# aligirayhanozbay/poisson_CNN

Measured on AMD Instinct MI355X. Metric: grids/sec (fwd+bwd) at 1024^2, higher is better.
Workload: dtype f32; 1 GPU; c4: Homogeneous_Poisson_NN_Legacy(hpnn.json) full train step (fwd+bwd+loss+Adam), 8 x 1024x1024 Dirichlet grids per GPU; global_batch=8, parallelism=dp1, math=fp32, ranks_seen=1

## Files before the change

### poisson_cnn_amd/csrc/conv_small.hip

```cpp
#include "pcnn_internal.h"
#include "conv_epilogue.h"

int pcnn_conv_small_fwd(pcnn_handle h, const pcnn_conv_desc* d, const float* x, const float* w, const float* bias, const float* bn_scale,
                        const float* bn_shift, const float* residual, float* y, float* act_out);
int pcnn_conv_small_wgrad(pcnn_handle h, const pcnn_conv_desc* d, const float* x, const float* dz, float* dw, void* workspace, size_t workspace_bytes);
bool pcnn_conv_fwd_takes_narrow_route(pcnn_handle h, const pcnn_conv_desc* d);
bool pcnn_conv_small_fwd_eligible(const pcnn_conv_desc* d);
bool pcnn_conv_small_wgrad_eligible(const pcnn_conv_desc* d);
size_t pcnn_conv_small_wgrad_workspace(const pcnn_conv_desc* d);

namespace {

constexpr int STH = 8, STW = 32;
__host__ __device__ constexpr int lds_stride(int CI) { return CI == 16 ? 20 : CI; }

struct SmallParams {
  const float* x; const float* wp; const float* bias; const float* bn_scale; const float* bn_shift; const float* res; float* y; float* act_out;
  unsigned* absmax;
  int N, H, W, Cin, ldx, Ho, Wo, Cout, ldy, pt, pl, pad_mode; float pad_value; int act; float alpha;
  int ld_res, ld_act, tiles_x, tiles_y, vec_in, vec_out;
  const float* gact = nullptr; float* y2 = nullptr; float* bpart = nullptr;
  int ld_gact = 0, ld_y2 = 0, gmode = 0; float galpha = 1.f;
};

// ... 507 lines not shown
    if (p.a1 && own) store_px(p.a1, gy, gx, acc);
    float* xs = X + ((r + 2) * XC + (c + 2)) * C;
    float s[C];
#pragma unroll
    for (int q = 0; q < Q; ++q) {
      const f32x4 xv = *reinterpret_cast<const f32x4*>(xs + 4 * q);
#pragma unroll
      for (int j = 0; j < 4; ++j) s[4 * q + j] = inside ? xv[j] + acc[4 * q + j] : 0.f;
      *reinterpret_cast<f32x4*>(xs + 4 * q) = (f32x4){s[4 * q], s[4 * q + 1], s[4 * q + 2], s[4 * q + 3]};
    }
    if (p.o1 && own) store_px(p.o1, gy, gx, s);
  }
  __syncthreads();
#pragma unroll 1
  for (int idx = threadIdx.x; idx < TH * STW; idx += 256) {
    const int r = idx >> 5, c = idx & 31, gy = y0 + r, gx = x0 + c;
    float acc[C];
#pragma unroll
    for (int o = 0; o < C; ++o) acc[o] = 0.f;
    stage_conv3<C>(X + ((r + 2) * XC + (c + 2)) * C, XC, p.w2, acc);
    bias_act(acc, p.b2);
    if (gy < p.H && gx < p.W) store_px(p.y, gy, gx, acc);
  }
}

template <int C, int TH>
void launch_stage(pcnn_handle h, StageParams p) {
  constexpr size_t lds = ((size_t)(TH + 6) * (STW + 6) + (size_t)(TH + 4) * (STW + 4)) * C * sizeof(float);
  set_lds(resnet3_stage_kernel<C, TH>, lds);
  p.tiles_x = pcnn_cdiv(p.W, STW); p.tiles_y = pcnn_cdiv(p.H, TH);
  hipLaunchKernelGGL((resnet3_stage_kernel<C, TH>), dim3((unsigned)(p.N * p.tiles_x * p.tiles_y)), dim3(256), lds, h->stream, p);
}

__global__ __launch_bounds__(256) void small_post_bias_kernel(const float* __restrict__ bpart, int64_t nblk, int CO, float* __restrict__ dbias) {
  __shared__ float red[256];
  const int ch = blockIdx.x, t = threadIdx.x;
  float a = 0.f;
  for (int64_t b = t; b < nblk; b += 256) a += bpart[b * CO + ch];
  red[t] = a;
  __syncthreads();
  for (int st = 128; st > 0; st >>= 1) { if (t < st) red[t] += red[t + st]; __syncthreads(); }
  if (t == 0) dbias[ch] = red[0];
}

}

static int pad4(int c) { return (c + 3) & ~3; }

bool pcnn_conv_small_fwd_eligible(const pcnn_conv_desc* d) {
  if (d->kh != d->kw || (d->kh != 3 && d->kh != 5) || d->Cin > 16 || d->Cout > 16) return false;
  if (d->kh == 5 && pad4(d->Cin) * pad4(d->Cout) > 16 * 16) return false;
  return true;
}

bool pcnn_conv_small_wgrad_eligible(const pcnn_conv_desc* d) {
  return d->kh == d->kw && (d->kh == 3 || d->kh == 5) && d->Cin <= 16 && d->Cout <= 16;
}

size_t pcnn_conv_small_wgrad_workspace(const pcnn_conv_desc* d) {
  return pcnn_conv_small_wgrad_eligible(d) ? (size_t)wgrad_splits(d) * d->kh * d->kw * d->Cin * d->Cout * sizeof(float) : 0;
}

static int small_fwd_impl(pcnn_handle h, const pcnn_conv_desc* d, const float* x, const float* w, const float* bias, const float* bn_scale,
                          const float* bn_shift, const float* residual, float* y, float* act_out, const pcnn_post_desc* post);

int pcnn_conv_small_fwd(pcnn_handle h, const pcnn_conv_desc* d, const float* x, const float* w, const float* bias, const float* bn_scale,
                        const float* bn_shift, const float* residual, float* y, float* act_out) {
  return small_fwd_impl(h, d, x, w, bias, bn_scale, bn_shift, residual, y, act_out, nullptr);
}

static bool quads_ok(const void* q, int ld) { return q == nullptr || pcnn_quads_ok(q, ld); }
extern "C" int pcnn_conv2d_dgrad_post_eligible(pcnn_handle h, const pcnn_conv_desc* dg, const float* dz, const float* residual, const float* dx, const pcnn_post_desc* post) {
  if (!h || !dg || !post || !post->act_out) return 0;
  if (dg->pad_mode != PCNN_PAD_CONSTANT || dg->act != PCNN_ACT_LINEAR || dg->N < 1) return 0;
  if (!pcnn_conv_small_fwd_eligible(dg) || !pcnn_conv_fwd_takes_narrow_route(h, dg)) return 0;
// ... 8 lines not shown
  return small_fwd_impl(h, dg, dz, w_flipped, nullptr, nullptr, nullptr, residual, dx, nullptr, post);
}

static int small_fwd_impl(pcnn_handle h, const pcnn_conv_desc* d, const float* x, const float* w, const float* bias, const float* bn_scale,
                          const float* bn_shift, const float* residual, float* y, float* act_out, const pcnn_post_desc* post) {
  const int CI = pad4(d->Cin), CO = pad4(d->Cout), taps = d->kh * d->kw;
  const size_t need = (size_t)taps * CI * CO * sizeof(float);
  if (pcnn_reserve(h, h->scratch, need, PCNN_SCRATCH_FLOOR, "pcnn_conv2d_fwd")) return 1;
  float* wp = static_cast<float*>(h->scratch.p);
  hipLaunchKernelGGL(pack_small_kernel, dim3(pcnn_cdiv(taps * CI * CO, 256)), dim3(256), 0, h->stream, w, wp, taps, d->Cin, d->Cout, CI, CO);
  SmallParams p;
  p.x = x; p.wp = wp; p.bias = bias; p.bn_scale = bn_scale; p.bn_shift = bn_shift; p.res = residual; p.y = y; p.act_out = act_out;
  p.absmax = reinterpret_cast<unsigned*>(h->y_absmax);
  p.N = d->N; p.H = d->H; p.W = d->W; p.Cin = d->Cin; p.ldx = d->ldx; p.Ho = d->Ho; p.Wo = d->Wo; p.Cout = d->Cout; p.ldy = d->ldy;
  p.pt = d->pad_top; p.pl = d->pad_left; p.pad_mode = d->pad_mode; p.pad_value = d->pad_value; p.act = d->act; p.alpha = d->act_alpha;
  p.ld_res = d->ld_res; p.ld_act = d->ld_act_out;
  p.tiles_x = pcnn_cdiv(d->Wo, STW); p.tiles_y = pcnn_cdiv(d->Ho, STH);
  p.vec_in = pcnn_quads_ok(x, d->ldx);
  p.vec_out = conv_epilogue_vec_ok(d->Cout, y, d->ldy, residual, d->ld_res, act_out, d->ld_act_out);
  const int64_t nblk = (int64_t)d->N * p.tiles_x * p.tiles_y;
  PCNN_REQUIRE(h, nblk < (1ll << 31), "pcnn_conv2d_fwd: grid too large");
  if (post) {
    p.gact = post->act_out; p.ld_gact = post->ld_act_out; p.y2 = post->raw_out; p.ld_y2 = post->ld_raw; p.gmode = post->act;
    p.galpha = post->act == PCNN_ACT_LINEAR ? 1.f : (post->act == PCNN_ACT_RELU ? 0.f : post->act_alpha);
    if (post->dbias) {
      if (pcnn_reserve(h, h->aux_ws, (size_t)nblk * CO * sizeof(float), 0, "pcnn_conv2d_dgrad_post")) return 1;
      p.bpart = static_cast<float*>(h->aux_ws.p);
    }
  }
  const bool ok = d->kh == 3 ? dispatch_ci<3>(h, p, nblk, CI, CO) : dispatch_ci<5>(h, p, nblk, CI, CO);
  PCNN_REQUIRE(h, ok, "pcnn_conv2d_fwd(small): no kernel for %d->%d", d->Cin, d->Cout);
  PCNN_CHECK_LAUNCH(h, "pcnn_conv2d_fwd(small)");
  if (post && post->dbias) {
    hipLaunchKernelGGL(small_post_bias_kernel, dim3((unsigned)d->Cout), dim3(256), 0, h->stream, p.bpart, nblk, CO, post->dbias);
    PCNN_CHECK_LAUNCH(h, "pcnn_conv2d_dgrad_post(bias)");
  }
  return 0;
}

int pcnn_conv_small_wgrad(pcnn_handle h, const pcnn_conv_desc* d, const float* x, const float* dz, float* dw, void* workspace, size_t workspace_bytes) {
  PCNN_REQUIRE(h, workspace_bytes >= pcnn_conv_small_wgrad_workspace(d), "pcnn_conv2d_wgrad(small): workspace too small");
  const int CI = pad4(d->Cin), CO = pad4(d->Cout);
  SmallWgradParams p;
  p.x = x; p.dz = dz; p.part = static_cast<float*>(workspace);
  p.N = d->N; p.H = d->H; p.W = d->W; p.Cin = d->Cin; p.ldx = d->ldx; p.Ho = d->Ho; p.Wo = d->Wo; p.Cout = d->Cout; p.lddz = d->ldy;
  p.pt = d->pad_top; p.pl = d->pad_left; p.pad_mode = d->pad_mode; p.pad_value = d->pad_value;
  p.tiles_x = pcnn_cdiv(d->Wo, STW); p.tiles_y = pcnn_cdiv(d->Ho, STH); p.ntiles = d->N * p.tiles_x * p.tiles_y; p.S = wgrad_splits(d);
  p.vec_in = pcnn_quads_ok(x, d->ldx);
  p.vec_dz = pcnn_quads_ok(dz, d->ldy);
  const bool ok = d->kh == 3 ? wgrad_dispatch_ci<3>(h, p, CI, CO) : wgrad_dispatch_ci<5>(h, p, CI, CO);
  PCNN_REQUIRE(h, ok, "pcnn_conv2d_wgrad(small): no kernel for %d->%d", d->Cin, d->Cout);
  PCNN_CHECK_LAUNCH(h, "pcnn_conv2d_wgrad(small)");
  const int nel = d->kh * d->kw * d->Cin * d->Cout;
  hipLaunchKernelGGL(small_wgrad_reduce_kernel, dim3(pcnn_cdiv(nel, 16)), dim3(256), 0, h->stream, p.part, dw, nel, p.S);
  PCNN_CHECK_LAUNCH(h, "pcnn_conv2d_wgrad(small reduce)");
  return 0;
}

extern "C" int pcnn_resnet3_fwd_eligible(pcnn_handle h, int C, int act) {
  return (h && (C == 4 || C == 8) && (act == PCNN_ACT_LINEAR || act == PCNN_ACT_RELU || act == PCNN_ACT_LEAKY_RELU)) ? 1 : 0;
}

extern "C" int pcnn_resnet3_fwd(pcnn_handle h, int N, int H, int W, int C, int act, float act_alpha, const float* x, const float* w0, const float* b0,
                                const float* w1, const float* b1, const float* w2, const float* b2, float* o0, float* a1, float* o1, float* y) {
  PCNN_REQUIRE(h, h && x && w0 && w1 && w2 && y, "pcnn_resnet3_fwd: null argument");
  PCNN_REQUIRE(h, pcnn_resnet3_fwd_eligible(h, C, act), "pcnn_resnet3_fwd: %d channels / activation %d are not eligible (ask pcnn_resnet3_fwd_eligible first)", C, act);
  PCNN_REQUIRE(h, N >= 1 && H >= 1 && W >= 1, "pcnn_resnet3_fwd: bad shape");
// ... 14 lines not shown
```

### poisson_cnn_amd/csrc/pointwise.hip

```cpp
#include "pcnn_internal.h"

namespace {

constexpr int CS_BLOCK = 256;
constexpr int CS_MAXBLK = 1024;

static int pow2_ge(int c) { int p = 1; while (p < c) p <<= 1; return p; }

__global__ __launch_bounds__(CS_BLOCK) void epilogue_bwd_kernel(int64_t npix, int C, int CP, const float* __restrict__ dy, int lddy,
                                                                const float* __restrict__ a, int lda, const float* __restrict__ bn_scale,
                                                                int act, float alpha, float* __restrict__ dz, int lddz,
                                                                float* __restrict__ partial , unsigned* __restrict__ absmax) {
  __shared__ float red[3][CS_BLOCK];
  const int tid = threadIdx.x, c = tid % CP, r = tid / CP, R = CS_BLOCK / CP;
  float s0 = 0.f, s1 = 0.f, s2 = 0.f, zmax = 0.f;
  if (c < C) {
    const float sc = bn_scale ? bn_scale[c] : 1.f;
    for (int64_t pix = (int64_t)blockIdx.x * R + r; pix < npix; pix += (int64_t)gridDim.x * R) {
      const float g = dy[pix * lddy + c];
      const float av = a ? a[pix * lda + c] : 0.f;
      const float z = g * sc * pcnn_act_grad_from_out(av, act, alpha);
      if (dz) dz[pix * lddz + c] = z;
      s0 += z; s1 += g * av; s2 += g; zmax = fmaxf(zmax, fabsf(z));
    }
// ... 211 lines not shown
  const int64_t total = npix * C;
  for (int64_t i = (int64_t)blockIdx.x * blockDim.x + threadIdx.x; i < total; i += (int64_t)gridDim.x * blockDim.x) {
    const int c = i % C; const int64_t pix = i / C;
    float* dst = &y[pix * ldy + c];
    const float v = alpha * x[pix * ldx + c];
    *dst = beta == 0.f ? v : v + beta * *dst;
  }
}

__global__ void assemble_input_kernel(int N, int H, int W, const float* __restrict__ rhs, int use_pos, float* __restrict__ out, int ldo) {
  const int64_t total = (int64_t)N * H * W;
  const float pi = 3.14159265358979323846f;
  for (int64_t i = (int64_t)blockIdx.x * blockDim.x + threadIdx.x; i < total; i += (int64_t)gridDim.x * blockDim.x) {
    const int x = i % W; const int y = (i / W) % H;
    out[i * ldo] = rhs[i];
    if (use_pos) {
      const float ly = H > 1 ? (float)y * (1.0f / (float)(H - 1)) : 0.f;
      const float lx = W > 1 ? (float)x * (1.0f / (float)(W - 1)) : 0.f;
      out[i * ldo + 1] = cosf(pi * ly);
      out[i * ldo + 2] = cosf(pi * lx);
    }
  }
}

__global__ void channel_scale_fwd_kernel(int N, int64_t hw, int C, const float* __restrict__ x, int ldx, const float* __restrict__ s,
                                         float* __restrict__ y, int ldy) {
  const int64_t total = (int64_t)N * hw * C;
  for (int64_t i = (int64_t)blockIdx.x * blockDim.x + threadIdx.x; i < total; i += (int64_t)gridDim.x * blockDim.x) {
    const int c = i % C; const int64_t pix = i / C; const int n = pix / hw;
    y[pix * ldy + c] = x[pix * ldx + c] * s[n * C + c];
  }
}

__global__ __launch_bounds__(CS_BLOCK) void channel_scale_bwd_kernel(int64_t hw, int C, int CP, const float* __restrict__ x, int ldx,
                                                                     const float* __restrict__ s, const float* __restrict__ dy, int lddy,
                                                                     float* __restrict__ dx, int lddx, float* __restrict__ partial,
                                                                     int gmode, float galpha, float* __restrict__ bpartial) {
  __shared__ float red[CS_BLOCK];
  const int n = blockIdx.y, tid = threadIdx.x, c = tid % CP, r = tid / CP, R = CS_BLOCK / CP;
  float acc = 0.f, bacc = 0.f;
  if (c < C) {
    const float sv = s[n * C + c];
    for (int64_t q = (int64_t)blockIdx.x * R + r; q < hw; q += (int64_t)gridDim.x * R) {
      const int64_t pix = (int64_t)n * hw + q;
      const float g = dy[pix * lddy + c], xv = x[pix * ldx + c];
      acc += g * xv;
      float v = g * sv;
      if (bpartial) {
        v *= gmode == PCNN_ACT_TANH ? 1.f - xv * xv : (xv > 0.f ? 1.f : galpha);
        bacc += v;
      }
      dx[pix * lddx + c] = v;
    }
  }
  red[tid] = acc;
  __syncthreads();
  if (r == 0 && c < C) {
    float t = 0.f;
    for (int q = 0; q < R; ++q) t += red[q * CP + c];
    partial[((int64_t)n * gridDim.x + blockIdx.x) * C + c] = t;
  }
  if (bpartial) {
    __syncthreads();
    red[tid] = bacc;
    __syncthreads();
    if (r == 0 && c < C) {
      float t = 0.f;
      for (int q = 0; q < R; ++q) t += red[q * CP + c];
      bpartial[((int64_t)n * gridDim.x + blockIdx.x) * C + c] = t;
    }
  }
}

__global__ void channel_scale_bias_final_kernel(const float* __restrict__ bpartial, int N, int nb, int C, float* __restrict__ dbias) {
  const int c = blockIdx.x * blockDim.x + threadIdx.x;
  if (c >= C) return;
  float t = 0.f;
  for (int i = 0; i < N * nb; ++i) t += bpartial[(int64_t)i * C + c];
  dbias[c] = t;
}

__global__ void channel_scale_final_kernel(const float* __restrict__ partial, int N, int nblk, int C, float* __restrict__ ds) {
  const int i = blockIdx.x * blockDim.x + threadIdx.x;
  if (i >= N * C) return;
  const int n = i / C, c = i % C;
  float t = 0.f;
  for (int b = 0; b < nblk; ++b) t += partial[((int64_t)n * nblk + b) * C + c];
  ds[i] = t;
}

__global__ void sample_scale_fwd_kernel(int N, int64_t per, const float* __restrict__ x, const float* __restrict__ g, float* __restrict__ y) {
  const int64_t total = (int64_t)N * per;
  for (int64_t i = (int64_t)blockIdx.x * blockDim.x + threadIdx.x; i < total; i += (int64_t)gridDim.x * blockDim.x)
    y[i] = x[i] * (1.0f + g[i / per]);
}

constexpr int SS_SPLIT = 64;
__global__ __launch_bounds__(256) void sample_scale_bwd_kernel(int64_t per, const float* __restrict__ x, const float* __restrict__ g,
                                                               const float* __restrict__ dy, float* __restrict__ dx, float* __restrict__ part) {
  __shared__ float red[256];
  const int n = blockIdx.y, sp = blockIdx.x;
  const float gv = 1.0f + g[n];
  const int64_t piece = (per + SS_SPLIT - 1) / SS_SPLIT, q0 = (int64_t)sp * piece, q1 = q0 + piece < per ? q0 + piece : per;
  float acc = 0.f;
  for (int64_t q = q0 + threadIdx.x; q < q1; q += blockDim.x) {
    const int64_t i = (int64_t)n * per + q;
    const float d = dy[i];
    acc += d * x[i];
    dx[i] = d * gv;
  }
  red[threadIdx.x] = acc;
  __syncthreads();
// ... 267 lines not shown
    for (int64_t i = (int64_t)blockIdx.x * blockDim.x + threadIdx.x; i < total; i += (int64_t)gridDim.x * blockDim.x) {
      const int c = i % C; int64_t r = i / C; const int xx = r % W; r /= W; const int yy = r % H; const int n = r / H;
      const bool hit = (yy % s == 0) && (xx % s == 0);
      y[(((int64_t)n * H + yy) * W + xx) * ldy + c] = hit ? x[(((int64_t)n * Ho + yy / s) * Wo + xx / s) * ldx + c] : 0.f;
    }
  }
}

extern "C" int pcnn_subsample(pcnn_handle h, int N, int H, int W, int C, int stride, const float* x, int ldx, float* y, int ldy, int adjoint) {
  PCNN_REQUIRE(h, h && x && y && stride >= 1 && N >= 1 && H >= 1 && W >= 1 && C >= 1, "pcnn_subsample: bad argument");
  const int Ho = (H + stride - 1) / stride, Wo = (W + stride - 1) / stride;
  hipLaunchKernelGGL(subsample_kernel, grid1d((int64_t)N * (adjoint ? (int64_t)H * W : (int64_t)Ho * Wo) * C), dim3(256), 0, h->stream, N, H, W, C, stride, Ho, Wo,
                     x, ldx, y, ldy, adjoint);
  PCNN_CHECK_LAUNCH(h, "pcnn_subsample");
  return 0;
}

extern "C" int pcnn_axpby(pcnn_handle h, int64_t npix, int C, float alpha, const float* x, int ldx, float beta, float* y, int ldy) {
  PCNN_REQUIRE(h, h && x && y, "pcnn_axpby: null argument");
  hipLaunchKernelGGL(axpby_kernel, grid1d(npix * C), dim3(256), 0, h->stream, npix, C, alpha, x, ldx, beta, y, ldy);
  PCNN_CHECK_LAUNCH(h, "pcnn_axpby");
  return 0;
}

extern "C" int pcnn_assemble_input(pcnn_handle h, int N, int H, int W, const float* rhs, int use_pos, float* out, int ldo) {
  PCNN_REQUIRE(h, h && rhs && out && ldo >= (use_pos ? 3 : 1), "pcnn_assemble_input: bad argument");
  hipLaunchKernelGGL(assemble_input_kernel, grid1d((int64_t)N * H * W), dim3(256), 0, h->stream, N, H, W, rhs, use_pos, out, ldo);
  PCNN_CHECK_LAUNCH(h, "pcnn_assemble_input");
  return 0;
}

extern "C" int pcnn_channel_scale_fwd(pcnn_handle h, int N, int64_t hw, int C, const float* x, int ldx, const float* s, float* y, int ldy) {
  PCNN_REQUIRE(h, h && x && s && y, "pcnn_channel_scale_fwd: null argument");
  hipLaunchKernelGGL(channel_scale_fwd_kernel, grid1d((int64_t)N * hw * C), dim3(256), 0, h->stream, N, hw, C, x, ldx, s, y, ldy);
  PCNN_CHECK_LAUNCH(h, "pcnn_channel_scale_fwd");
  return 0;
}

static int cs_blocks(int64_t hw, int CP) {
  int64_t nb = pcnn_cdiv64(hw, (int64_t)(CS_BLOCK / CP) * 16);
  if (nb > 256) nb = 256;
  if (nb < 1) nb = 1;
  return (int)nb;
}

extern "C" size_t pcnn_channel_scale_workspace(int N, int64_t hw, int C) { return (size_t)N * 256 * (size_t)C * sizeof(float); }

extern "C" int pcnn_channel_scale_bwd(pcnn_handle h, int N, int64_t hw, int C, const float* x, int ldx, const float* s, const float* dy, int lddy,
                                      float* dx, int lddx, float* ds, void* workspace, size_t workspace_bytes) {
  PCNN_REQUIRE(h, h && x && s && dy && dx && ds && workspace, "pcnn_channel_scale_bwd: null argument");
  PCNN_REQUIRE(h, C >= 1 && C <= CS_BLOCK, "pcnn_channel_scale_bwd: C=%d unsupported", C);
  PCNN_REQUIRE(h, workspace_bytes >= pcnn_channel_scale_workspace(N, hw, C), "pcnn_channel_scale_bwd: workspace too small");
  const int CP = pow2_ge(C), nb = cs_blocks(hw, CP);
  float* partial = static_cast<float*>(workspace);
  hipLaunchKernelGGL(channel_scale_bwd_kernel, dim3(nb, N), dim3(CS_BLOCK), 0, h->stream, hw, C, CP, x, ldx, s, dy, lddy, dx, lddx, partial, 0, 1.f, (float*)nullptr);
  PCNN_CHECK_LAUNCH(h, "pcnn_channel_scale_bwd");
  hipLaunchKernelGGL(channel_scale_final_kernel, dim3(pcnn_cdiv(N * C, 128)), dim3(128), 0, h->stream, partial, N, nb, C, ds);
  PCNN_CHECK_LAUNCH(h, "pcnn_channel_scale_bwd(final)");
  return 0;
}

extern "C" int pcnn_channel_scale_bwd_post(pcnn_handle h, int N, int64_t hw, int C, const float* x, int ldx, const float* s, const float* dy, int lddy,
                                           float* dz, int lddz, float* ds, int act, float act_alpha, float* dbias, void* workspace, size_t workspace_bytes) {
  PCNN_REQUIRE(h, h && x && s && dy && dz && ds && workspace, "pcnn_channel_scale_bwd_post: null argument");
  PCNN_REQUIRE(h, C >= 1 && C <= CS_BLOCK, "pcnn_channel_scale_bwd_post: C=%d unsupported", C);
  PCNN_REQUIRE(h, act == PCNN_ACT_LINEAR || act == PCNN_ACT_RELU || act == PCNN_ACT_LEAKY_RELU || act == PCNN_ACT_TANH, "pcnn_channel_scale_bwd_post: activation %d", act);
  PCNN_REQUIRE(h, workspace_bytes >= 2 * pcnn_channel_scale_workspace(N, hw, C), "pcnn_channel_scale_bwd_post: workspace too small");
  const int CP = pow2_ge(C), nb = cs_blocks(hw, CP);
  float* partial = static_cast<float*>(workspace);
  float* bpartial = partial + (size_t)N * 256 * C;
  const float galpha = act == PCNN_ACT_LINEAR ? 1.f : (act == PCNN_ACT_RELU ? 0.f : act_alpha);
  hipLaunchKernelGGL(channel_scale_bwd_kernel, dim3(nb, N), dim3(CS_BLOCK), 0, h->stream, hw, C, CP, x, ldx, s, dy, lddy, dz, lddz, partial, act, galpha, bpartial);
  PCNN_CHECK_LAUNCH(h, "pcnn_channel_scale_bwd_post");
  hipLaunchKernelGGL(channel_scale_final_kernel, dim3(pcnn_cdiv(N * C, 128)), dim3(128), 0, h->stream, partial, N, nb, C, ds);
  if (dbias) hipLaunchKernelGGL(channel_scale_bias_final_kernel, dim3(pcnn_cdiv(C, 64)), dim3(64), 0, h->stream, bpartial, N, nb, C, dbias);
  PCNN_CHECK_LAUNCH(h, "pcnn_channel_scale_bwd_post(final)");
  return 0;
}

extern "C" int pcnn_sample_scale_fwd(pcnn_handle h, int N, int64_t per, const float* x, const float* g, float* y) {
  PCNN_REQUIRE(h, h && x && g && y, "pcnn_sample_scale_fwd: null argument");
  hipLaunchKernelGGL(sample_scale_fwd_kernel, grid1d((int64_t)N * per), dim3(256), 0, h->stream, N, per, x, g, y);
  PCNN_CHECK_LAUNCH(h, "pcnn_sample_scale_fwd");
  return 0;
}

extern "C" int pcnn_sample_scale_bwd(pcnn_handle h, int N, int64_t per, const float* x, const float* g, const float* dy, float* dx, float* dg) {
  PCNN_REQUIRE(h, h && x && g && dy && dx && dg, "pcnn_sample_scale_bwd: null argument");
  const size_t need = (size_t)N * SS_SPLIT * sizeof(float);
  if (pcnn_reserve(h, h->aux_ws, need, (size_t)1 << 20, "pcnn_sample_scale_bwd")) return 1;
  float* part = static_cast<float*>(h->aux_ws.p);
  hipLaunchKernelGGL(sample_scale_bwd_kernel, dim3(SS_SPLIT, N), dim3(256), 0, h->stream, per, x, g, dy, dx, part);
  hipLaunchKernelGGL(sample_scale_final_kernel, dim3((N + 63) / 64), dim3(64), 0, h->stream, N, part, dg);
  PCNN_CHECK_LAUNCH(h, "pcnn_sample_scale_bwd");
  return 0;
}

extern "C" int pcnn_bc_ring_fwd(pcnn_handle h, int N, int H, int W, int neumann, const float* x, float* y) {
  PCNN_REQUIRE(h, h && x && y, "pcnn_bc_ring_fwd: null argument");
  PCNN_REQUIRE(h, H >= 3 && W >= 3, "pcnn_bc_ring_fwd: grid %dx%d too small", H, W);
  hipLaunchKernelGGL(bc_ring_fwd_kernel, grid1d((int64_t)N * H * W), dim3(256), 0, h->stream, N, H, W, neumann, x, y);
  PCNN_CHECK_LAUNCH(h, "pcnn_bc_ring_fwd");
  return 0;
}

extern "C" int pcnn_bc_ring_edges_fwd(pcnn_handle h, int N, int H, int W, int neumann_mask, const float* x, float* y) {
  PCNN_REQUIRE(h, h && x && y, "pcnn_bc_ring_edges_fwd: null argument");
  PCNN_REQUIRE(h, H >= 3 && W >= 3, "pcnn_bc_ring_edges_fwd: grid %dx%d too small", H, W);
// ... 272 lines not shown
```

### poisson_cnn_amd/csrc/spectral_conv.hip

```cpp
#include "spectral_common.h"
#include <math.h>
#include <stdlib.h>
#include <array>
#include <vector>

int pcnn_spectral_conv_fwd(pcnn_handle h, const pcnn_conv_desc* d, const float* x, const float* w, const float* bias, const float* bn_scale,
                           const float* bn_shift, const float* residual, float* y, float* act_out);
int pcnn_spectral_conv_wgrad(pcnn_handle h, const pcnn_conv_desc* d, const float* x, const float* dz, float* dw);
bool pcnn_spectral_eligible(pcnn_handle h, const pcnn_conv_desc* d, bool wgrad);
bool pcnn_conv_small_fwd_eligible(const pcnn_conv_desc* d);
bool pcnn_conv_fwd_takes_narrow_route(pcnn_handle h, const pcnn_conv_desc* d);

using namespace pcnn_spec;


namespace {

constexpr int T = 32, ROWS = 1024, NSLOT = 512;
constexpr int TAB_G = 0, TAB_GI = 1024, TAB_F2 = 2048, TAB_FI2 = 4096, TAB_GI2 = 6144, TAB_FLOATS = TAB32_FLOATS;
static_assert(TAB_GI2 + 1024 == TAB_FLOATS, "table block");
constexpr size_t LDS_U = (size_t)T * T * 32 * sizeof(float);
constexpr size_t LDS_INV = LDS_U + 1024 * sizeof(float);
__host__ __device__ __forceinline__ int64_t sp_item(int64_t item) { return pcnn_spec::sp_item(item, ROWS); }

// ... 360 lines not shown
  load_a(mt, 0, a);
  auto m_tile = [&](int mt) {
    f32x16 acc[3] = {zero16(), zero16(), zero16()};
#pragma unroll
    for (int gi = 0; gi < GIN; ++gi) {
      if (gi + 1 < GIN) load_a(mt, gi + 1, an);
      else if (mt + mstride < nMt) load_a(mt + mstride, 0, an);
#pragma unroll
      for (int j = 0; j < 16; ++j) {
        const float xr = a[0][j >> 2][j & 3], xi = a[1][j >> 2][j & 3];
        acc[0] = mfma(fmaf(s_cplx, xi, xr), b1[gi][j], acc[0]);
        acc[1] = mfma(real2 ? xi : xr, b2[gi][j], acc[1]);
        acc[2] = mfma(xi, b3[gi][j], acc[2]);
      }
#pragma unroll
      for (int pp = 0; pp < 2; ++pp)
#pragma unroll
        for (int j4 = 0; j4 < 4; ++j4) a[pp][j4] = an[pp][j4];
    }
#pragma unroll
    for (int r = 0; r < 16; ++r) {
      const int trow = mt * 32 + acc_row(r, half);
      float* o = &p.ys[pcnn_spec::sp_item((int64_t)trow * p.gout + go, p.rows) + c];
      o[rr * RS] = acc[0][r] + acc[2][r];
      o[ri * RS] = fmaf(s_cplx, acc[0][r], acc[1][r]);
    }
  };
  m_tile(mt);
  for (mt += mstride; mt < nMt; mt += mstride) m_tile(mt);
}

struct WMixParams { const float* xs; const float* ds; float* part; const int4* slots; int ntile, gin, S, accumulate, rows, nslot; };

__global__ __launch_bounds__(256, 2) void spec_wmix_kernel(WMixParams p) {
  const int tid = threadIdx.x, lane = tid & 63, half = lane >> 5, c = lane & 31;
  const int wave = __builtin_amdgcn_readfirstlane(tid >> 6);
  const int slot = blockIdx.x, gi = blockIdx.z;
  const int part = blockIdx.y * 4 + wave, nparts = p.S * 4;
  const int4 sl = p.slots[slot];
  const int per = (((p.ntile + nparts - 1) / nparts) + 1) & ~1;
  const int t0 = part * per, t1 = min(t0 + per, p.ntile);
  const float* xr = p.xs + sl.x * RS, *xi = p.xs + sl.y * RS;
  const float* dr = p.ds + sl.x * RS, *di = p.ds + sl.y * RS;
  int kind = sl.z;
  asm volatile("" : "+v"(kind));
  const float s_cplx = kind == 1 ? 0.f : 1.f;
  f32x16 acc[3] = {zero16(), zero16(), zero16()};
  constexpr int WU = 4;
  float ar[WU], ai[WU], br[WU], bi[WU], nar[WU], nai[WU], nbr[WU], nbi[WU];
  auto load = [&](int tb, float (&a0)[WU], float (&a1)[WU], float (&b0)[WU], float (&b1)[WU]) {
#pragma unroll
    for (int u = 0; u < WU; ++u) {
      const int tt = tb + 2 * u + half;
      const unsigned tc = (unsigned)(tt < t1 ? tt : t0);
      const unsigned ix = (unsigned)pcnn_spec::sp_item((int64_t)tc * p.gin + gi, p.rows) + c, id = (unsigned)pcnn_spec::sp_item(tc, p.rows) + c;
      a0[u] = __builtin_nontemporal_load(&xr[ix]); a1[u] = __builtin_nontemporal_load(&xi[ix]); b0[u] = __builtin_nontemporal_load(&dr[id]); b1[u] = __builtin_nontemporal_load(&di[id]);
    }
  };
  if (t0 < t1) load(t0, ar, ai, br, bi);
  for (int tb = t0; tb < t1; tb += 2 * WU) {
    if (tb + 2 * WU < t1) load(tb + 2 * WU, nar, nai, nbr, nbi);
#pragma unroll
    for (int u = 0; u < WU; ++u) {
      const bool ok = tb + 2 * u + half < t1;
      const float a0 = ok ? ar[u] : 0.f, a1 = ok ? ai[u] : 0.f;
      acc[0] = mfma(fmaf(-s_cplx, a1, a0), br[u], acc[0]);
      acc[1] = mfma(a0, bi[u] - br[u], acc[1]);
      acc[2] = mfma(a1, fmaf(s_cplx, br[u], bi[u]), acc[2]);
    }
#pragma unroll
    for (int u = 0; u < WU; ++u) { ar[u] = nar[u]; ai[u] = nai[u]; br[u] = nbr[u]; bi[u] = nbi[u]; }
  }
  float* o = p.part + (((int64_t)part * p.nslot + slot) * p.gin + gi) * 4 * 1024 + c;
#pragma unroll
  for (int qd = 0; qd < 3; ++qd) {
    float old[16];
    if (p.accumulate) {
#pragma unroll
      for (int r = 0; r < 16; ++r) old[r] = o[qd * 1024 + acc_row(r, half) * 32];
    }
#pragma unroll
    for (int r = 0; r < 16; ++r) o[qd * 1024 + acc_row(r, half) * 32] = p.accumulate ? old[r] + acc[qd][r] : acc[qd][r];
  }
}

struct MixWParams { const float* zs; const float* xs; float* ys; float* part; const float* wsp; const int4* slots; int ntile, gx, rows, nslot, Cz, cpt, accumulate; };

__global__ __launch_bounds__(256, 2) void spec_mixw_kernel(MixWParams p) {
  const int tid = threadIdx.x, lane = tid & 63, half = lane >> 5, c = lane & 31;
  const int wave = __builtin_amdgcn_readfirstlane(tid >> 6);
  const int slot = blockIdx.x, g = blockIdx.z;
  const int part = blockIdx.y * 4 + wave;
  const int4 sl = p.slots[slot];
  const int rr = sl.x, ri = sl.y;
  float hr[16], hi[16];
  const bool real2 = sl.z == 1;
  const float s_neg = real2 ? 0.f : -1.f, s_pos = real2 ? 0.f : 1.f;
  int kind = sl.z;
  asm volatile("" : "+v"(kind));
  const float s_cplx = kind == 1 ? 0.f : 1.f;
  {
    const int co = c % p.cpt;
#pragma unroll
    for (int j = 0; j < 16; ++j) {
      const int kc = j + 16 * half, ci = kc % p.cpt;
      float wr = 0.f, wi = 0.f;
      if (ci < p.Cz && kc / p.cpt == c / p.cpt) {
        const float* wg = p.wsp + pcnn_spec::sp_item(ci * p.gx + g, p.rows) + co;
        wr = wg[rr * RS]; wi = wg[ri * RS];
      }
      hr[j] = wr; hi[j] = wi;
    }
  }
  const int nMt = (p.ntile + 31) >> 5;
  const int mstride = gridDim.y * 4;
  const float* xr = p.xs + rr * RS, *xi = p.xs + ri * RS;
// ... 46 lines not shown
        const int j = 8 * (qu & 1) + e;
        const float av = aq[qu & 1][e >> 2][e & 3];
        if (qu < 2) {
          acc[0] = mfma(av, hr[j], acc[0]);
          acc[1] = mfma(av * s_neg, hi[j], acc[1]);
        } else {
          acc[0] = mfma(av * s_pos, hi[j], acc[0]);
          acc[1] = mfma(av, real2 ? hi[j] : hr[j], acc[1]);
        }
      }
    };
    mfma_w(mt, 0, ws[0]); load_w(mt, 2, ws[0]);     __builtin_amdgcn_sched_barrier(0);
    mix_quarter(0);       load_a_part(mt, 1, 0);    __builtin_amdgcn_sched_barrier(0);
    mfma_w(mt, 1, ws[1]); load_w(mt, 3, ws[1]);     __builtin_amdgcn_sched_barrier(0);
    mix_quarter(1);       load_a_part(mt, 1, 1);    __builtin_amdgcn_sched_barrier(0);
    mfma_w(mt, 2, ws[0]); load_w(mn, 0, ws[0]);     __builtin_amdgcn_sched_barrier(0);
    mix_quarter(2);       load_a_part(mn, 0, 0);    __builtin_amdgcn_sched_barrier(0);
    mfma_w(mt, 3, ws[1]); load_w(mn, 1, ws[1]);     __builtin_amdgcn_sched_barrier(0);
    mix_quarter(3);       load_a_part(mn, 0, 1);    __builtin_amdgcn_sched_barrier(0);
#pragma unroll
    for (int nt = 0; nt < 2; ++nt) {
      const int row = nt ? ri : rr;
#pragma unroll
      for (int r = 0; r < 16; ++r) {
        const int trow = mt * 32 + acc_row(r, half);
        p.ys[pcnn_spec::sp_item((int64_t)trow * p.gx + g, p.rows) + row * RS + c] = acc[nt][r];
      }
    }
  };
  if (mt < nMt) {
    m_tile(mt);
    for (mt += mstride; mt < nMt; mt += mstride) m_tile(mt);
  }
  float* o = p.part + (((int64_t)part * p.nslot + slot) * p.gx + g) * 4 * 1024 + c;
#pragma unroll
  for (int qd = 0; qd < 3; ++qd) {
    float old[16];
    if (p.accumulate) {
#pragma unroll
      for (int r = 0; r < 16; ++r) old[r] = o[qd * 1024 + acc_row(r, half) * 32];
    }
#pragma unroll
    for (int r = 0; r < 16; ++r) o[qd * 1024 + acc_row(r, half) * 32] = p.accumulate ? old[r] + accp[qd][r] : accp[qd][r];
  }
}

__global__ __launch_bounds__(256) void spec_wcombine_kernel(const float* __restrict__ part, const int4* __restrict__ slots, float* __restrict__ csp, int S, int gin, int Cin, float isign, int cpt, int rows) {
  const int nslot = rows / 2;
  const int slot = blockIdx.x, gi = blockIdx.y;
  const int4 sl = slots[slot];
  for (int e = threadIdx.x; e < 1024; e += 256) {
    const int cil = e >> 5, co = e & 31, ci = gi * 32 + cil;
    if (ci >= Cin || cil >= cpt || co >= cpt) continue;
    float P[3] = {0.f, 0.f, 0.f};
    for (int s = 0; s < S; ++s)
      for (int sub = 0; sub < 32 / cpt; ++sub) {
        const float* b = part + (((int64_t)s * nslot + slot) * gin + gi) * 4 * 1024 + (sub * cpt + cil) * 32 + sub * cpt + co;
#pragma unroll
        for (int qd = 0; qd < 3; ++qd) P[qd] += b[qd * 1024];
      }
    const float cr = sl.z == 1 ? P[0] : P[0] + P[2], cim = sl.z == 1 ? P[2] : -isign * (P[0] + P[1]);
    csp[pcnn_spec::sp_item(ci, rows) + sl.x * RS + co] = cr;
    csp[pcnn_spec::sp_item(ci, rows) + sl.y * RS + co] = cim;
  }
}

void build_tables(std::vector<float>& tab, std::vector<int>& slots) {
  tab.assign(TAB_FLOATS, 0.f);
  const double tp = 2.0 * M_PI / T;
  auto G = [&](int s, int x) { return s <= 16 ? cos(tp * s * x) : -sin(tp * (s - 16) * x); };
  auto Gi = [&](int n, int s) {
    if (s == 0) return 1.0 / T;
    if (s == 16) return ((n & 1) ? -1.0 : 1.0) / T;
    return s < 16 ? 2.0 * cos(tp * s * n) / T : -2.0 * sin(tp * (s - 16) * n) / T;
  };
  auto F2 = [&](int par, int row, int k) {
    const int po = row >> 4, m = row & 15, pi = k >> 4, y = k & 15;
// ... 363 lines not shown
  int chunk = std::min(chunk_tiles(g.T) / (gin > gout ? gin : gout), g.ntile);
  float* ws[3];
  if (int rc = carve_workspace(h, &chunk, [&](int ch) {
        return std::array<size_t, 3>{sp_region((size_t)d->Cin * gout, g.rows), sp_region((size_t)ch * gin, g.rows), sp_region((size_t)pad32(ch) * gout, g.rows)};
      }, ws)) return rc;
  float *wsp = ws[0], *xs = ws[1], *ys = ws[2];
  const Xform xf = xform_of(h, g.T);
  const float* fsp = filter_spectrum(h, xf, w, wsp, d->kh, d->kw, d->Cin, d->Cout, gout);
  PCNN_CHECK_LAUNCH(h, "spectral convolution (filter spectrum)");
  FwdParams fx = image_fwd_params(g, x, xs, d->H, d->W, d->Cin, d->ldx, gin, d->pad_top, d->pad_left, d->pad_mode, d->pad_value);
  InvParams iv = image_inv_params(g, ys, y, d->Ho, d->Wo, d->Cout, d->ldy, gout, residual, d->ld_res);
  iv.bias = bias; iv.bn_scale = bn_scale; iv.bn_shift = bn_shift; iv.act_out = act_out; iv.ld_act = d->ld_act_out;
  iv.absmax = reinterpret_cast<unsigned*>(h->y_absmax); iv.act = d->act; iv.alpha = d->act_alpha;
  MixParams mx;
  mx.xs = xs; mx.ys = ys; mx.wsp = fsp; mx.gin = gin; mx.gout = gout; mx.Cin = d->Cin; mx.cpt = g.cpt;
  for (int t0 = 0; t0 < g.ntile; t0 += chunk) {
    const int nt = std::min(chunk, g.ntile - t0);
    fx.tile0 = t0; iv.tile0 = t0;
    launch_fwd(h, xf, fx, nt);
    launch_mix(h, xf, mx, gin, gout, nt);
    launch_inv(h, xf, iv, nt);
  }
  PCNN_CHECK_LAUNCH(h, "spectral convolution");
  return 0;
}

int pcnn_spectral_conv_wgrad(pcnn_handle h, const pcnn_conv_desc* d, const float* x, const float* dz, float* dw) {
  TileGrid g;
  if (int rc = tile_grid(h, d, d->kh, d->kw, d->N, d->Ho, d->Wo, d->Cin, d->Cout, &g)) return rc;
  const int gin = pcnn_cdiv(d->Cin, 32), S = wgrad_splits(g.T);
  int chunk = std::min(chunk_tiles(g.T) / gin, g.ntile);
  float* ws[4];
  if (int rc = carve_workspace(h, &chunk, [&](int ch) {
        return std::array<size_t, 4>{sp_region((size_t)d->Cin, g.rows), sp_region((size_t)ch * gin, g.rows), sp_region((size_t)ch, g.rows), align256((size_t)S * g.nslot * gin * 4 * 1024 * 4)};
      }, ws)) return rc;
  float *csp = ws[0], *xs = ws[1], *zs = ws[2], *part = ws[3];
  const Xform xf = xform_of(h, g.T);
  FwdParams fx = image_fwd_params(g, x, xs, d->H, d->W, d->Cin, d->ldx, gin, d->pad_top, d->pad_left, d->pad_mode, d->pad_value);
  FwdParams fz = image_fwd_params(g, dz, zs, d->Ho, d->Wo, d->Cout, d->ldy, 1, 0, 0, PCNN_PAD_CONSTANT, 0.f);
  fz.ylim = g.Vy; fz.xlim = g.Vx;
  WMixParams wm;
  wm.xs = xs; wm.ds = zs; wm.part = part; wm.slots = xf.slots; wm.gin = gin; wm.S = S / 4; wm.rows = g.rows; wm.nslot = g.nslot;
  for (int t0 = 0; t0 < g.ntile; t0 += chunk) {
    const int nt = std::min(chunk, g.ntile - t0);
    fx.tile0 = t0; fz.tile0 = t0; wm.ntile = nt; wm.accumulate = t0 > 0;
    launch_fwd(h, xf, fx, nt);
    launch_fwd(h, xf, fz, nt);
    hipLaunchKernelGGL(spec_wmix_kernel, dim3(g.nslot, S / 4, gin), dim3(256), 0, h->stream, wm);
  }
  hipLaunchKernelGGL(spec_wcombine_kernel, dim3(g.nslot, gin), dim3(256), 0, h->stream, part, xf.slots, csp, S, gin, d->Cin, 1.0f, g.cpt, g.rows);
  launch_inv(h, xf, taps_params(xf, csp, dw, d->kh, d->kw, d->Cin, d->Cout, 0), 1);
  PCNN_CHECK_LAUNCH(h, "spectral weight gradient");
  return 0;
}

__global__ __launch_bounds__(256) void spec_canonical_rows_kernel(const float* __restrict__ sp, float* __restrict__ out, int T, int rows, int P) {
  const int item = blockIdx.y;
  for (int e = blockIdx.x * 256 + threadIdx.x; e < rows * 32; e += gridDim.x * 256) {
    const int r = e >> 5, c = e & 31;
    out[(size_t)item * rows * 32 + e] = sp[pcnn_spec::sp_item(item, rows) + pcnn_spec::sp_row_from_canonical(T, r, P) * RS + c];
  }
}
static int canonical_copy(pcnn_handle h, const Xform& xf, const float* sp, float* out, int items) {
  hipLaunchKernelGGL(spec_canonical_rows_kernel, dim3(16, items), dim3(256), 0, h->stream, sp, out, xf.T, xf.rows, xf.P);
  return hipGetLastError() == hipSuccess ? 0 : 1;
}

extern "C" int pcnn_debug_tile_spectrum64(pcnn_handle h, int H, int W, int C, const float* x, int ylim, int xlim, float* out) {
  PCNN_REQUIRE(h, h && x && out && H >= 1 && W >= 1 && C >= 1 && C <= 64, "pcnn_debug_tile_spectrum64: bad argument");
  TileGrid g;
  if (int rc = tile_grid_given(h, 64, 64, 64, 1, 1, 64, 64, &g)) return rc;
  const int groups = pcnn_cdiv(C, 32);
  char* r;
  if (int rc = ensure_workspace(h, sp_region((size_t)groups, g.rows), &r)) return rc;
  const Xform xf = xform_of(h, g.T);
  FwdParams f = image_fwd_params(g, x, reinterpret_cast<float*>(r), H, W, C, C, groups, 0, 0, PCNN_PAD_CONSTANT, 0.f);
  f.ylim = ylim; f.xlim = xlim;
  launch_fwd(h, xf, f, 1);
  PCNN_CHECK_LAUNCH(h, "pcnn_debug_tile_spectrum64");
  if (canonical_copy(h, xf, f.sp, out, groups)) PCNN_FAIL(h, "pcnn_debug_tile_spectrum64: copy failed");
  return 0;
}

// ... 33 lines not shown
  return d->Cin <= 32 ? 1 : 0;
}

static int bwd_spectral_impl(pcnn_handle h, const pcnn_conv_desc* d, const pcnn_conv_desc* dg, const float* x, const float* dz, const float* w_flipped,
                             const float* residual, float* dx, float* dw, const pcnn_post_desc* post);

extern "C" int pcnn_conv2d_bwd_spectral(pcnn_handle h, const pcnn_conv_desc* d, const pcnn_conv_desc* dg, const float* x, const float* dz, const float* w_flipped,
                                        const float* residual, float* dx, float* dw) {
  return bwd_spectral_impl(h, d, dg, x, dz, w_flipped, residual, dx, dw, nullptr);
}

extern "C" int pcnn_conv2d_bwd_spectral_post(pcnn_handle h, const pcnn_conv_desc* d, const pcnn_conv_desc* dg, const float* x, const float* dz, const float* w_flipped,
                                             const float* residual, float* dx, float* dw, const pcnn_post_desc* post) {
  PCNN_REQUIRE(h, h && post && post->act_out, "pcnn_conv2d_bwd_spectral_post: null argument");
  PCNN_REQUIRE(h, pcnn_conv2d_bwd_spectral_post_eligible(h, d, dg), "pcnn_conv2d_bwd_spectral_post: layer is not eligible (ask pcnn_conv2d_bwd_spectral_post_eligible first)");
  return bwd_spectral_impl(h, d, dg, x, dz, w_flipped, residual, dx, dw, post);
}

static int bwd_spectral_impl(pcnn_handle h, const pcnn_conv_desc* d, const pcnn_conv_desc* dg, const float* x, const float* dz, const float* w_flipped,
                             const float* residual, float* dx, float* dw, const pcnn_post_desc* post) {
  PCNN_REQUIRE(h, h && d && dg && x && dz && w_flipped && dx && dw, "pcnn_conv2d_bwd_spectral: null argument");
  if (pcnn_check_conv_desc(h, "pcnn_conv2d_bwd_spectral", d, 64, 32, PCNN_ANY) || pcnn_check_conv_desc(h, "pcnn_conv2d_bwd_spectral (dg)", dg, 32, 64, PCNN_ANY)) return 1;
  PCNN_REQUIRE(h, pcnn_conv2d_bwd_spectral_eligible(h, d, dg), "pcnn_conv2d_bwd_spectral: layer is not eligible (ask pcnn_conv2d_bwd_spectral_eligible first)");
  PCNN_REQUIRE(h, dg->Cin == d->Cout && dg->Cout == d->Cin && dg->kh == d->kh && dg->kw == d->kw && dg->N == d->N, "pcnn_conv2d_bwd_spectral: descriptors do not match");
  TileGrid g;
  if (int rc = tile_grid(h, dg, d->kh, d->kw, d->N, dg->Ho, dg->Wo, d->Cin, d->Cout, &g)) return rc;
  const int gz = 1, gx = pcnn_cdiv(d->Cin, 32), S = wgrad_splits(g.T);
  const size_t bs_b = post ? (size_t)POST_SLOTS_MAX * 64 * sizeof(float) : 0;
  int chunk = std::min(chunk_tiles(g.T) / gx, g.ntile);
  float* ws[7];
  if (int rc = carve_workspace(h, &chunk, [&](int ch) {
        const size_t ys_b = sp_region((size_t)pad32(ch) * gx, g.rows);
        return std::array<size_t, 7>{sp_region((size_t)std::max(dg->Cin * gx, d->Cin), g.rows), sp_region((size_t)ch * gz, g.rows), ys_b, ys_b,
                                     align256((size_t)S * g.nslot * gx * 4 * 1024 * 4), bs_b, 4096};
      }, ws)) return rc;
  float *wsp = ws[0], *zs = ws[1], *ys = ws[2], *xs = ws[3], *part = ws[4], *bsum = ws[5];
  const Xform xf = xform_of(h, g.T);
  PCNN_REQUIRE(h, gx == 1 || dg->Cout == 64, "pcnn_conv2d_bwd_spectral: %d input channels unsupported (<= 32 or 64)", d->Cin);
  const float* fsp = filter_spectrum(h, xf, w_flipped, wsp, d->kh, d->kw, dg->Cin, dg->Cout, gx);
  PCNN_CHECK_LAUNCH(h, "pcnn_conv2d_bwd_spectral (filter spectrum)");
  FwdParams fz = image_fwd_params(g, dz, zs, dg->H, dg->W, dg->Cin, dg->ldx, gz, dg->pad_top, dg->pad_left, dg->pad_mode, dg->pad_value);
  const bool padded_domain = d->pad_mode != PCNN_PAD_CONSTANT;
  FwdParams fxm = image_fwd_params(g, x, xs, d->H, d->W, d->Cin, d->ldx, gx, padded_domain ? d->pad_top : 0, padded_domain ? d->pad_left : 0, d->pad_mode, 0.f);
  fxm.ylim = g.Vy; fxm.xlim = g.Vx; fxm.ext_y = dg->Ho; fxm.ext_x = dg->Wo;
  InvParams iv = image_inv_params(g, ys, dx, dg->Ho, dg->Wo, dg->Cout, dg->ldy, gx, residual, dg->ld_res);
  if (post) {
    iv.gact = post->act_out; iv.ld_gact = post->ld_act_out; iv.gmode = post->act; iv.galpha = post->act_alpha;
    iv.y2 = post->raw_out; iv.ld_y2 = post->ld_raw; iv.bsum = post->dbias ? bsum : nullptr;
    if (iv.bsum && hipMemsetAsync(bsum, 0, bs_b, h->stream) != hipSuccess) PCNN_FAIL(h, "pcnn_conv2d_bwd_spectral_post: memset failed");
  }
  MixWParams mw;
  mw.zs = zs; mw.xs = xs; mw.ys = ys; mw.part = part; mw.wsp = fsp; mw.slots = xf.slots; mw.gx = gx; mw.rows = g.rows; mw.nslot = g.nslot;
  mw.Cz = dg->Cin; mw.cpt = g.cpt;
  for (int t0 = 0; t0 < g.ntile; t0 += chunk) {
    const int nt = std::min(chunk, g.ntile - t0);
    fz.tile0 = t0; fxm.tile0 = t0; iv.tile0 = t0; mw.ntile = nt; mw.accumulate = t0 > 0;
    launch_fwd(h, xf, fz, nt);
    launch_fwd(h, xf, fxm, nt);
    hipLaunchKernelGGL(spec_mixw_kernel, dim3(g.nslot, S / 4, gx), dim3(256), 0, h->stream, mw);
    launch_inv(h, xf, iv, nt);
  }
  if (post && post->dbias) xf.post_bias(h, bsum, g.pack, g.cpt, dg->Cout, post->dbias);
  float* csp = wsp;
  hipLaunchKernelGGL(spec_wcombine_kernel, dim3(g.nslot, gx), dim3(256), 0, h->stream, part, xf.slots, csp, S, gx, d->Cin, -1.0f, g.cpt, g.rows);
  launch_inv(h, xf, taps_params(xf, csp, dw, d->kh, d->kw, d->Cin, d->Cout, 1), 1);
  PCNN_CHECK_LAUNCH(h, "pcnn_conv2d_bwd_spectral");
  return 0;
}
```

Measured before the change: 43.44 grids/s.

## Reduce spectral wgrad partials in LDS, vectorize channel scale and bias reductions

```diff
diff --git a/poisson_cnn_amd/csrc/conv_small.hip b/poisson_cnn_amd/csrc/conv_small.hip
--- a/poisson_cnn_amd/csrc/conv_small.hip
+++ b/poisson_cnn_amd/csrc/conv_small.hip
@@ -563,15 +563,24 @@
   hipLaunchKernelGGL((resnet3_stage_kernel<C, TH>), dim3((unsigned)(p.N * p.tiles_x * p.tiles_y)), dim3(256), lds, h->stream, p);
 }
 
-__global__ __launch_bounds__(256) void small_post_bias_kernel(const float* __restrict__ bpart, int64_t nblk, int CO, float* __restrict__ dbias) {
-  __shared__ float red[256];
-  const int ch = blockIdx.x, t = threadIdx.x;
-  float a = 0.f;
-  for (int64_t b = t; b < nblk; b += 256) a += bpart[b * CO + ch];
+constexpr int PB_BLOCK = 1024;
+__global__ __launch_bounds__(PB_BLOCK) void small_post_bias_kernel(const float* __restrict__ bpart, int64_t nblk, int CO, int Cout, float* __restrict__ dbias) {
+  __shared__ f32x4 red[PB_BLOCK];
+  const int t = threadIdx.x, Q = CO >> 2, R = PB_BLOCK / Q, r = t / Q, q = t - r * Q;
+  f32x4 a = {0.f, 0.f, 0.f, 0.f};
+  if (r < R) {
+#pragma unroll 8
+    for (int64_t b = r; b < nblk; b += R) a += *reinterpret_cast<const f32x4*>(bpart + b * CO + 4 * q);
+  }
   red[t] = a;
   __syncthreads();
-  for (int st = 128; st > 0; st >>= 1) { if (t < st) red[t] += red[t + st]; __syncthreads(); }
-  if (t == 0) dbias[ch] = red[0];
+  int st = 1;
+  while (st < R) st <<= 1;
+  for (st >>= 1; st > 0; st >>= 1) {
+    if (r < st && r + st < R) red[t] += red[t + st * Q];
+    __syncthreads();
+  }
+  if (t < Cout) dbias[t] = red[t >> 2][t & 3];
 }
 
 }
@@ -646,7 +655,7 @@
   PCNN_REQUIRE(h, ok, "pcnn_conv2d_fwd(small): no kernel for %d->%d", d->Cin, d->Cout);
   PCNN_CHECK_LAUNCH(h, "pcnn_conv2d_fwd(small)");
   if (post && post->dbias) {
-    hipLaunchKernelGGL(small_post_bias_kernel, dim3((unsigned)d->Cout), dim3(256), 0, h->stream, p.bpart, nblk, CO, post->dbias);
+    hipLaunchKernelGGL(small_post_bias_kernel, dim3(1), dim3(PB_BLOCK), 0, h->stream, p.bpart, nblk, CO, d->Cout, post->dbias);
     PCNN_CHECK_LAUNCH(h, "pcnn_conv2d_dgrad_post(bias)");
   }
   return 0;
diff --git a/poisson_cnn_amd/csrc/pointwise.hip b/poisson_cnn_amd/csrc/pointwise.hip
--- a/poisson_cnn_amd/csrc/pointwise.hip
+++ b/poisson_cnn_amd/csrc/pointwise.hip
@@ -267,6 +267,21 @@
   }
 }
 
+__global__ __launch_bounds__(256) void channel_scale_fwd_vec4_kernel(int64_t hw, int C, const float* __restrict__ x, int ldx, const float* __restrict__ s,
+                                                                     float* __restrict__ y, int ldy) {
+  const int Q = C >> 2, R = 256 / Q, tid = threadIdx.x, r = tid / Q, q = tid - r * Q, n = blockIdx.y;
+  if (r >= R) return;
+  const float* sn = s + (int64_t)n * C + 4 * q;
+  const float s0 = sn[0], s1 = sn[1], s2 = sn[2], s3 = sn[3];
+  const float* xn = x + (int64_t)n * hw * ldx + 4 * q;
+  float* yn = y + (int64_t)n * hw * ldy + 4 * q;
+#pragma unroll 4
+  for (int64_t p = (int64_t)blockIdx.x * R + r; p < hw; p += (int64_t)gridDim.x * R) {
+    const float4 v = *reinterpret_cast<const float4*>(xn + p * ldx);
+    *reinterpret_cast<float4*>(yn + p * ldy) = make_float4(v.x * s0, v.y * s1, v.z * s2, v.w * s3);
+  }
+}
+
 __global__ __launch_bounds__(CS_BLOCK) void channel_scale_bwd_kernel(int64_t hw, int C, int CP, const float* __restrict__ x, int ldx,
                                                                      const float* __restrict__ s, const float* __restrict__ dy, int lddy,
                                                                      float* __restrict__ dx, int lddx, float* __restrict__ partial,
@@ -307,12 +322,24 @@
   }
 }
 
-__global__ void channel_scale_bias_final_kernel(const float* __restrict__ bpartial, int N, int nb, int C, float* __restrict__ dbias) {
-  const int c = blockIdx.x * blockDim.x + threadIdx.x;
-  if (c >= C) return;
+constexpr int BF_BLOCK = 1024;
+__global__ __launch_bounds__(BF_BLOCK) void channel_scale_bias_final_kernel(const float* __restrict__ bpartial, int rows, int C, float* __restrict__ dbias) {
+  __shared__ float red[BF_BLOCK];
+  const int tid = threadIdx.x, R = BF_BLOCK / C, r = tid / C, c = tid - r * C;
   float t = 0.f;
-  for (int i = 0; i < N * nb; ++i) t += bpartial[(int64_t)i * C + c];
-  dbias[c] = t;
+  if (r < R) {
+#pragma unroll 8
+    for (int i = r; i < rows; i += R) t += bpartial[(int64_t)i * C + c];
+  }
+  red[tid] = t;
+  __syncthreads();
+  int st = 1;
+  while (st < R) st <<= 1;
+  for (st >>= 1; st > 0; st >>= 1) {
+    if (r + st < R && r < st) red[tid] += red[tid + st * C];
+    __syncthreads();
+  }
+  if (tid < C) dbias[tid] = red[tid];
 }
 
 __global__ void channel_scale_final_kernel(const float* __restrict__ partial, int N, int nblk, int C, float* __restrict__ ds) {
@@ -646,7 +673,13 @@
 
 extern "C" int pcnn_channel_scale_fwd(pcnn_handle h, int N, int64_t hw, int C, const float* x, int ldx, const float* s, float* y, int ldy) {
   PCNN_REQUIRE(h, h && x && s && y, "pcnn_channel_scale_fwd: null argument");
-  hipLaunchKernelGGL(channel_scale_fwd_kernel, grid1d((int64_t)N * hw * C), dim3(256), 0, h->stream, N, hw, C, x, ldx, s, y, ldy);
+  if (C >= 4 && C % 4 == 0 && C <= 1024 && N >= 1 && N <= 65535 && hw >= 1 && pcnn_quads_ok(x, ldx) && pcnn_quads_ok(y, ldy)) {
+    const int R = 256 / (C / 4);
+    const int64_t nb = std::min<int64_t>(pcnn_cdiv64(hw, (int64_t)R * 4), 2048);
+    hipLaunchKernelGGL(channel_scale_fwd_vec4_kernel, dim3((unsigned)nb, (unsigned)N), dim3(256), 0, h->stream, hw, C, x, ldx, s, y, ldy);
+  } else {
+    hipLaunchKernelGGL(channel_scale_fwd_kernel, grid1d((int64_t)N * hw * C), dim3(256), 0, h->stream, N, hw, C, x, ldx, s, y, ldy);
+  }
   PCNN_CHECK_LAUNCH(h, "pcnn_channel_scale_fwd");
   return 0;
 }
@@ -687,7 +720,7 @@
   hipLaunchKernelGGL(channel_scale_bwd_kernel, dim3(nb, N), dim3(CS_BLOCK), 0, h->stream, hw, C, CP, x, ldx, s, dy, lddy, dz, lddz, partial, act, galpha, bpartial);
   PCNN_CHECK_LAUNCH(h, "pcnn_channel_scale_bwd_post");
   hipLaunchKernelGGL(channel_scale_final_kernel, dim3(pcnn_cdiv(N * C, 128)), dim3(128), 0, h->stream, partial, N, nb, C, ds);
-  if (dbias) hipLaunchKernelGGL(channel_scale_bias_final_kernel, dim3(pcnn_cdiv(C, 64)), dim3(64), 0, h->stream, bpartial, N, nb, C, dbias);
+  if (dbias) hipLaunchKernelGGL(channel_scale_bias_final_kernel, dim3(1), dim3(BF_BLOCK), 0, h->stream, bpartial, N * nb, C, dbias);
   PCNN_CHECK_LAUNCH(h, "pcnn_channel_scale_bwd_post(final)");
   return 0;
 }
diff --git a/poisson_cnn_amd/csrc/spectral_conv.hip b/poisson_cnn_amd/csrc/spectral_conv.hip
--- a/poisson_cnn_amd/csrc/spectral_conv.hip
+++ b/poisson_cnn_amd/csrc/spectral_conv.hip
@@ -416,6 +416,32 @@
 
 struct WMixParams { const float* xs; const float* ds; float* part; const int4* slots; int ntile, gin, S, accumulate, rows, nslot; };
 
+
+__device__ __forceinline__ void store_wave_sums(const f32x16 (&acc)[3], float* __restrict__ out, int accumulate) {
+  __shared__ float wsum[3 * 1024];
+  const int tid = threadIdx.x, lane = tid & 63, half = lane >> 5, c = lane & 31, wave = tid >> 6;
+#pragma unroll
+  for (int w = 0; w < 4; ++w) {
+    if (wave == w) {
+#pragma unroll
+      for (int qd = 0; qd < 3; ++qd)
+#pragma unroll
+        for (int r = 0; r < 16; ++r) {
+          float* d = &wsum[qd * 1024 + acc_row(r, half) * 32 + c];
+          *d = w == 0 ? acc[qd][r] : *d + acc[qd][r];
+        }
+    }
+    __syncthreads();
+  }
+  float old[12];
+  if (accumulate) {
+#pragma unroll
+    for (int i = 0; i < 12; ++i) old[i] = out[i * 256 + tid];
+  }
+#pragma unroll
+  for (int i = 0; i < 12; ++i) out[i * 256 + tid] = accumulate ? old[i] + wsum[i * 256 + tid] : wsum[i * 256 + tid];
+}
+
 __global__ __launch_bounds__(256, 2) void spec_wmix_kernel(WMixParams p) {
   const int tid = threadIdx.x, lane = tid & 63, half = lane >> 5, c = lane & 31;
   const int wave = __builtin_amdgcn_readfirstlane(tid >> 6);
@@ -455,17 +481,7 @@
 #pragma unroll
     for (int u = 0; u < WU; ++u) { ar[u] = nar[u]; ai[u] = nai[u]; br[u] = nbr[u]; bi[u] = nbi[u]; }
   }
-  float* o = p.part + (((int64_t)part * p.nslot + slot) * p.gin + gi) * 4 * 1024 + c;
-#pragma unroll
-  for (int qd = 0; qd < 3; ++qd) {
-    float old[16];
-    if (p.accumulate) {
-#pragma unroll
-      for (int r = 0; r < 16; ++r) old[r] = o[qd * 1024 + acc_row(r, half) * 32];
-    }
-#pragma unroll
-    for (int r = 0; r < 16; ++r) o[qd * 1024 + acc_row(r, half) * 32] = p.accumulate ? old[r] + acc[qd][r] : acc[qd][r];
-  }
+  store_wave_sums(acc, p.part + (((int64_t)blockIdx.y * p.nslot + slot) * p.gin + gi) * 4 * 1024, p.accumulate);
 }
 
 struct MixWParams { const float* zs; const float* xs; float* ys; float* part; const float* wsp; const int4* slots; int ntile, gx, rows, nslot, Cz, cpt, accumulate; };
@@ -578,17 +594,7 @@
     m_tile(mt);
     for (mt += mstride; mt < nMt; mt += mstride) m_tile(mt);
   }
-  float* o = p.part + (((int64_t)part * p.nslot + slot) * p.gx + g) * 4 * 1024 + c;
-#pragma unroll
-  for (int qd = 0; qd < 3; ++qd) {
-    float old[16];
-    if (p.accumulate) {
-#pragma unroll
-      for (int r = 0; r < 16; ++r) old[r] = o[qd * 1024 + acc_row(r, half) * 32];
-    }
-#pragma unroll
-    for (int r = 0; r < 16; ++r) o[qd * 1024 + acc_row(r, half) * 32] = p.accumulate ? old[r] + accp[qd][r] : accp[qd][r];
-  }
+  store_wave_sums(accp, p.part + (((int64_t)blockIdx.y * p.nslot + slot) * p.gx + g) * 4 * 1024, p.accumulate);
 }
 
 __global__ __launch_bounds__(256) void spec_wcombine_kernel(const float* __restrict__ part, const int4* __restrict__ slots, float* __restrict__ csp, int S, int gin, int Cin, float isign, int cpt, int rows) {
@@ -1018,7 +1024,7 @@
   int chunk = std::min(chunk_tiles(g.T) / gin, g.ntile);
   float* ws[4];
   if (int rc = carve_workspace(h, &chunk, [&](int ch) {
-        return std::array<size_t, 4>{sp_region((size_t)d->Cin, g.rows), sp_region((size_t)ch * gin, g.rows), sp_region((size_t)ch, g.rows), align256((size_t)S * g.nslot * gin * 4 * 1024 * 4)};
+        return std::array<size_t, 4>{sp_region((size_t)d->Cin, g.rows), sp_region((size_t)ch * gin, g.rows), sp_region((size_t)ch, g.rows), align256((size_t)(S / 4) * g.nslot * gin * 4 * 1024 * 4)};
       }, ws)) return rc;
   float *csp = ws[0], *xs = ws[1], *zs = ws[2], *part = ws[3];
   const Xform xf = xform_of(h, g.T);
@@ -1034,7 +1040,7 @@
     launch_fwd(h, xf, fz, nt);
     hipLaunchKernelGGL(spec_wmix_kernel, dim3(g.nslot, S / 4, gin), dim3(256), 0, h->stream, wm);
   }
-  hipLaunchKernelGGL(spec_wcombine_kernel, dim3(g.nslot, gin), dim3(256), 0, h->stream, part, xf.slots, csp, S, gin, d->Cin, 1.0f, g.cpt, g.rows);
+  hipLaunchKernelGGL(spec_wcombine_kernel, dim3(g.nslot, gin), dim3(256), 0, h->stream, part, xf.slots, csp, S / 4, gin, d->Cin, 1.0f, g.cpt, g.rows);
   launch_inv(h, xf, taps_params(xf, csp, dw, d->kh, d->kw, d->Cin, d->Cout, 0), 1);
   PCNN_CHECK_LAUNCH(h, "spectral weight gradient");
   return 0;
@@ -1134,7 +1140,7 @@
   if (int rc = carve_workspace(h, &chunk, [&](int ch) {
         const size_t ys_b = sp_region((size_t)pad32(ch) * gx, g.rows);
         return std::array<size_t, 7>{sp_region((size_t)std::max(dg->Cin * gx, d->Cin), g.rows), sp_region((size_t)ch * gz, g.rows), ys_b, ys_b,
-                                     align256((size_t)S * g.nslot * gx * 4 * 1024 * 4), bs_b, 4096};
+                                     align256((size_t)(S / 4) * g.nslot * gx * 4 * 1024 * 4), bs_b, 4096};
       }, ws)) return rc;
   float *wsp = ws[0], *zs = ws[1], *ys = ws[2], *xs = ws[3], *part = ws[4], *bsum = ws[5];
   const Xform xf = xform_of(h, g.T);
@@ -1164,7 +1170,7 @@
   }
   if (post && post->dbias) xf.post_bias(h, bsum, g.pack, g.cpt, dg->Cout, post->dbias);
   float* csp = wsp;
-  hipLaunchKernelGGL(spec_wcombine_kernel, dim3(g.nslot, gx), dim3(256), 0, h->stream, part, xf.slots, csp, S, gx, d->Cin, -1.0f, g.cpt, g.rows);
+  hipLaunchKernelGGL(spec_wcombine_kernel, dim3(g.nslot, gx), dim3(256), 0, h->stream, part, xf.slots, csp, S / 4, gx, d->Cin, -1.0f, g.cpt, g.rows);
   launch_inv(h, xf, taps_params(xf, csp, dw, d->kh, d->kw, d->Cin, d->Cout, 1), 1);
   PCNN_CHECK_LAUNCH(h, "pcnn_conv2d_bwd_spectral");
   return 0;
```

Result: no change. 43.78 grids/s, median of 6 (+0.8%).
